# nl1xx/simple-multimodal

Hardware: AMD Instinct MI355X
Metric: fusion fwd+bwd samples/sec at B=16 d=768 (higher is better)
Workload: dtype bf16

## Files before the change

simple-multimodal_amd/csrc/gemm7.hip:

```cpp
#include <algorithm>
#include <vector>
#include "gemm6_parts.h"

namespace {

constexpr int BK = 32, NS = 4;
constexpr int TILE = 256 * BK * 2, PPO = BK / 8;
template <int TN> struct Form {
  static constexpr int BNT = 64 * TN, TILE_B = BNT * BK * 2, STAGE = TILE + TILE_B, PPB = TN, PPW = PPO + PPB;
  static constexpr int LDS = NS * STAGE + 4 * 8192;
};
static_assert(Form<4>::LDS == 160 * 1024 && Form<3>::LDS == 144 * 1024, "LDS of the two forms");

typedef int i32x4_t __attribute__((ext_vector_type(4)));

struct TileSrc {
  const unsigned short* Ab;
  const unsigned short* Bb;
  int recA, recB, stepB, KT;
};
struct TileDst {
  int pi, m0, n0;
};

__device__ __forceinline__ int to_sgpr(int x) {
  int r;
  asm volatile("s_nop 0\n\tv_readfirstlane_b32 %0, %1\n\ts_nop 4" : "=s"(r) : "v"(x));
  return r;
}

template <bool B_KR, int TN>
__device__ __forceinline__ void locate_tile(const GemmArgs& args, const int total_tiles, const int orig, TileSrc& s, TileDst& d, int& lda, int& ldb) {
  const int bid = to_sgpr(mmf_xcd_tile(orig, total_tiles, args.xcd_granule));
  int pi = 0;
  while (pi + 1 < args.nprob && bid >= args.tile_start[pi + 1]) ++pi;
  const mmf_gemm_problem& P = args.p[pi];
  int m0, n0;
  tile_origin<Form<TN>::BNT>(P, bid - args.tile_start[pi], m0, n0);
  m0 = to_sgpr(m0);
  n0 = to_sgpr(n0);
  d.pi = pi; d.m0 = m0; d.n0 = n0;
  lda = P.lda; ldb = P.ldb;
  s.Ab = static_cast<const unsigned short*>(P.A) + (size_t)m0 * P.lda;
  s.Bb = static_cast<const unsigned short*>(P.B) + (B_KR ? (size_t)n0 : (size_t)n0 * P.ldb);
  s.recA = (int)(((long)(P.M - m0 - 1) * P.lda + P.K) * 2);
  s.recB = (int)((B_KR ? ((long)(P.K - 1) * P.ldb + (P.N - n0)) : ((long)(P.N - n0 - 1) * P.ldb + P.K)) * 2);
  s.stepB = (B_KR ? BK * P.ldb : BK) * 2;
  s.KT = P.K / BK;
}

template <int CT, int TN>
__device__ __forceinline__ void drain_tile(const GemmArgs& args, const int pi, const mmf_gemm_problem& P, const int mb, const int nb,
                                           f32x16_t (&acc)[TN][4], char* region, const int lane) {
  constexpr bool AUX = (CT & (MMF_EPI_MASK_AUX | MMF_EPI_ADD_AUX)) != 0;
  constexpr bool DROP = (CT & MMF_EPI_DROPOUT) != 0;
  const unsigned drop_key = DROP ? mmf_rng_key(*args.rng_state, args.site, (unsigned)args.orig[pi]) : 0u;
  const float drop_scale = DROP ? 1.f / (1.f - (float)args.drop_thresh * (1.f / 4294967296.f)) : 1.f;
  const float alpha = (CT & MMF_EPI_MASK_AUX) ? args.alpha : 1.f;
  const int r = lane & 31, h = lane >> 5, q = lane >> 4, cq = lane & 15;
  const unsigned wr_base = (unsigned)(r * 256 + 8 * h + 16 * (r & 15));
  const unsigned rd_base = (unsigned)(q * 256 + ((cq ^ q) << 4));
  auto acc_at = [&](int c) { return region + (wr_base ^ (unsigned)(c << 4)); };
  auto row_at = [&](int it) { return region + it * 1024 + (rd_base ^ (unsigned)((it & 3) << 6)); };
  const bool col_ok = cq < 4 * TN && nb + 8 * cq < P.N;
  const __amdgpu_buffer_rsrc_t crs = __builtin_amdgcn_make_buffer_rsrc(P.C, 0, (int)((((long)P.M - 1) * P.ldc + P.N) * 2), 0x00020000);
  const __amdgpu_buffer_rsrc_t ars = __builtin_amdgcn_make_buffer_rsrc(const_cast<void*>(AUX ? P.aux : P.C), 0,
                                                                       AUX ? (int)((((long)P.M - 1) * P.ldaux + P.N) * 2) : 0, 0x00020000);
  const unsigned c_off0 = col_ok ? (unsigned)(((long)(mb + q) * P.ldc + nb + 8 * cq) * 2) : 0x80000000u;
  const unsigned a_off0 = col_ok ? (unsigned)(((long)(mb + q) * P.ldaux + nb + 8 * cq) * 2) : 0x80000000u;
  const unsigned c_row4 = (unsigned)(4 * P.ldc * 2), a_row4 = (unsigned)(4 * P.ldaux * 2);

  u32x4_t auxr[2][8];
  auto load_aux = [&](int tm, int slot) {
#pragma unroll
    for (int it = 0; it < 8; ++it)
      auxr[slot][it] = __builtin_bit_cast(u32x4_t, __builtin_amdgcn_raw_buffer_load_b128(ars, a_off0 + (unsigned)(8 * tm + it) * a_row4, 0, 0));
  };
  if constexpr (AUX) { load_aux(0, 0); load_aux(1, 1); }
#pragma unroll
  for (int tm = 0; tm < 4; ++tm) {
    u32x2_t axv[TN][4];
    if constexpr (AUX) {
#pragma unroll
      for (int it = 0; it < 8; ++it) *reinterpret_cast<u32x4_t*>(row_at(it)) = auxr[tm & 1][it];
#pragma unroll
      for (int tn = 0; tn < TN; ++tn)
#pragma unroll
        for (int g = 0; g < 4; ++g) axv[tn][g] = *reinterpret_cast<const u32x2_t*>(acc_at(4 * tn + g));
      __builtin_amdgcn_sched_barrier(0);
      if (tm + 2 < 4) load_aux(tm + 2, tm & 1);
      __builtin_amdgcn_sched_barrier(0);
    }
#pragma unroll
    for (int tn = 0; tn < TN; ++tn) {
      asm volatile("" : "+a"(acc[tn][tm]));
#pragma unroll
      for (int g = 0; g < 4; ++g) {
        f32x4_t v = {acc[tn][tm][4 * g], acc[tn][tm][4 * g + 1], acc[tn][tm][4 * g + 2], acc[tn][tm][4 * g + 3]};
        if constexpr (CT & MMF_EPI_RELU) {
#pragma unroll
          for (int e = 0; e < 4; ++e) v[e] = fmaxf(v[e], 0.f);
        }
        if constexpr (DROP) {
          const unsigned idx = (unsigned)(mb + 32 * tm + r) * (unsigned)P.N + (unsigned)(nb + 32 * tn + 8 * g + 4 * h);
#pragma unroll
          for (int e = 0; e < 4; ++e) v[e] = mmf_keep(drop_key, idx + e, args.drop_thresh) ? v[e] * drop_scale : 0.f;
        }
        if constexpr (AUX) {
          const u32x2_t a = axv[tn][g];
          const float a0 = bf16lo(a[0]), a1 = bf16hi(a[0]), a2 = bf16lo(a[1]), a3 = bf16hi(a[1]);
          if constexpr (CT & MMF_EPI_MASK_AUX) {
            v[0] = a0 > 0.f ? v[0] * alpha : 0.f; v[1] = a1 > 0.f ? v[1] * alpha : 0.f;
            v[2] = a2 > 0.f ? v[2] * alpha : 0.f; v[3] = a3 > 0.f ? v[3] * alpha : 0.f;
          } else {
            v[0] += a0; v[1] += a1; v[2] += a2; v[3] += a3;
          }
        }
        *reinterpret_cast<u32x2_t*>(acc_at(4 * tn + g)) = u32x2_t{pack_bf16x2(v[0], v[1]), pack_bf16x2(v[2], v[3])};
      }
      __builtin_amdgcn_sched_barrier(0);
    }
    u32x4_t w[8];
#pragma unroll
    for (int it = 0; it < 8; ++it) w[it] = *reinterpret_cast<const u32x4_t*>(row_at(it));
#pragma unroll
    for (int it = 0; it < 8; ++it) __builtin_amdgcn_raw_buffer_store_b128(w[it], crs, c_off0 + (unsigned)(8 * tm + it) * c_row4, 0, 0);
    __builtin_amdgcn_sched_barrier(0);
  }
}

template <bool B_KR, int CT, int TN>
__device__ __forceinline__ void gemm7_body(const GemmArgs& args, const int total_tiles, char* smem) {
  constexpr bool A_KR = false;
  using F = Form<TN>;
  constexpr int BNT = F::BNT, STAGE = F::STAGE, PPW = F::PPW, NMF = 4 * TN, NRD = 4 + TN;
  constexpr int WA = BK, WB = B_KR ? BNT : BK;

  const int tid = threadIdx.x, lane = tid & 63;
  const int wave = __builtin_amdgcn_readfirstlane(tid >> 6);
  const int wm = wave >> 1, wn = wave & 1;
  const int nwg = gridDim.x;
  const int wid = blockIdx.x;
  auto walk = [&](int round) { return round * nwg + ((round & 1) ? nwg - 1 - wid : wid); };
  int round = 0;
  int orig = walk(0);
  TileSrc ns;
  TileDst cd, nd;
  int KT, lda, ldb;
  locate_tile<B_KR, TN>(args, total_tiles, orig, ns, cd, lda, ldb);
  KT = ns.KT;

  unsigned voff[PPW], voffn[PPW];
  auto set_voff = [&](unsigned (&v)[PPW], int la, int lb) {
#pragma unroll
    for (int i = 0; i < PPO; ++i) v[i] = piece_voff<A_KR, BK>(wave + 4 * i, la, lane);
#pragma unroll
    for (int i = 0; i < TN; ++i) v[PPO + i] = piece_voff<B_KR, BK, BNT>(wave + 4 * i, lb, lane);
  };
  set_voff(voff, lda, ldb);
  char* const my_pieces = smem + wave * 1024;

  struct Desc { int lo, hi, rec; };
  auto mkdesc = [](const unsigned short* p, int rec) {
    const unsigned long long a = (unsigned long long)(uintptr_t)p;
    return Desc{(int)(unsigned)a, (int)((unsigned)(a >> 32) & 0xffffu), rec};
  };
  auto advance = [](Desc& d, int bytes) {
    const unsigned long long a = (((unsigned long long)(unsigned)d.hi << 32) | (unsigned)d.lo) + (unsigned long long)bytes;
    d.lo = (int)(unsigned)a; d.hi = (int)(unsigned)(a >> 32);
    int r;
    asm("s_sub_i32 %0, %1, %2\n\ts_max_i32 %0, %0, 0" : "=s"(r) : "s"(d.rec), "s"(bytes) : "scc");
    d.rec = r;
  };
  Desc dA = mkdesc(ns.Ab, ns.recA);
  Desc dB = mkdesc(ns.Bb, ns.recB);
  constexpr int stepA = BK * 2;
  int stepB = ns.stepB;
  const unsigned lds_pieces = (unsigned)(uintptr_t)(const __attribute__((address_space(3))) char*)my_pieces;
  auto hot_piece = [&](auto ic, const unsigned ring_base) {
    constexpr int I = decltype(ic)::value, OFF = I < PPO ? I * 4096 : TILE + (I - PPO) * 4096;
    const Desc& d = I < PPO ? dA : dB;
    const i32x4_t q = {d.lo, d.hi, d.rec, 0x00020000};
    int m0w;
    asm volatile("s_add_i32 %0, %1, %4\n\ts_nop 0\n\tbuffer_load_dwordx4 %2, %3, 0 offen lds" : "={m0}"(m0w) : "s"(ring_base), "v"(voff[I]), "s"(q), "n"(OFF) : "memory");
    __builtin_amdgcn_sched_barrier(0);
  };

#pragma unroll
  for (int s = 0; s < NS; ++s) {
    const unsigned rb = lds_pieces + (unsigned)(s * STAGE);
    hot_piece(std::integral_constant<int, 0>{}, rb); hot_piece(std::integral_constant<int, 1>{}, rb);
    hot_piece(std::integral_constant<int, 2>{}, rb); hot_piece(std::integral_constant<int, 3>{}, rb);
    if (s + 1 < NS) {
      hot_piece(std::integral_constant<int, 4>{}, rb); hot_piece(std::integral_constant<int, 5>{}, rb);
      hot_piece(std::integral_constant<int, 6>{}, rb);
      if constexpr (TN == 4) hot_piece(std::integral_constant<int, 7>{}, rb);
      advance(dA, stepA); advance(dB, stepB);
    }
  }

  bool has_next = walk(1) < total_tiles;
  nd = cd;
  if (has_next) {
    int la, lb;
    locate_tile<B_KR, TN>(args, total_tiles, walk(1), ns, nd, la, lb);
    set_voff(voffn, la, lb);
  } else {
    ns.recA = 0; ns.recB = 0; ns.stepB = 0;
#pragma unroll
    for (int i = 0; i < PPW; ++i) voffn[i] = voff[i];
  }

  unsigned la0, la1, lb0, lb1;
  Frag4<A_KR>::lane_parts(WA, lane, la0, la1);
  Frag4<B_KR>::lane_parts(WB, lane, lb0, lb1);
  const unsigned smem_base = (unsigned)(uintptr_t)(const __attribute__((address_space(3))) char*)smem;
  const unsigned qa = (unsigned)((WA / 32) * 2048 * 4 * wm);
  const unsigned qb = (unsigned)(B_KR ? 512 * TN * wn : (WB / 32) * 2048 * TN * wn);
  la0 += smem_base + qa; la1 += smem_base + qa;
  lb0 += smem_base + TILE + qb; lb1 += smem_base + TILE + qb;

  f32x16_t acc[TN][4];

  constexpr bool use_bias = (CT & MMF_EPI_BIAS) != 0;
  float bcur[TN] = {};
  auto load_bias = [&](float (&b)[TN], const TileDst& d) {
    const mmf_gemm_problem& P = args.p[d.pi];
    const __amdgpu_buffer_rsrc_t brs = __builtin_amdgcn_make_buffer_rsrc(const_cast<float*>(P.bias), 0, P.N * 4, 0x00020000);
    const unsigned off = (unsigned)((d.n0 + 32 * TN * wn + (lane & 31)) * 4);
#pragma unroll
    for (int tn = 0; tn < TN; ++tn)
      b[tn] = __uint_as_float((unsigned)__builtin_amdgcn_raw_buffer_load_b32(brs, off + (unsigned)(32 * tn * 4), 0, 0));
  };
  auto split3 = [&](float x) {
    const bool lo = lane < 32;
    const unsigned hh = __float_as_uint(x) & 0xffff0000u;
    const float r1 = x - __uint_as_float(hh);
    const unsigned mm = __float_as_uint(r1) & 0xffff0000u;
    const float r2 = r1 - __uint_as_float(mm);
    const unsigned ll = __float_as_uint(r2) & 0xffff0000u;
    const u32x4_t w = {lo ? ((hh >> 16) | mm) : 0u, lo ? (ll >> 16) : 0u, 0u, 0u};
    return __builtin_bit_cast(bf16x8_t, w);
  };
  auto bias_init = [&](const float (&b)[TN]) {
    const f32x16_t zero = {0.f, 0.f, 0.f, 0.f, 0.f, 0.f, 0.f, 0.f, 0.f, 0.f, 0.f, 0.f, 0.f, 0.f, 0.f, 0.f};
    const u32x4_t ow = {lane < 32 ? 0x3f803f80u : 0u, lane < 32 ? 0x00003f80u : 0u, 0u, 0u};
    u32x4_t ones[4] = {ow, ow, ow, ow};
#pragma unroll
    for (int tm = 0; tm < 4; ++tm) asm volatile("" : "+v"(ones[tm]));
#pragma unroll
    for (int tn = 0; tn < TN; ++tn) {
      u32x4_t bw = __builtin_bit_cast(u32x4_t, use_bias ? split3(b[tn]) : __builtin_bit_cast(bf16x8_t, u32x4_t{0u, 0u, 0u, 0u}));
      asm volatile("" : "+v"(bw));
#pragma unroll
      for (int tm = 0; tm < 4; ++tm) {
        acc[tn][tm] = __builtin_amdgcn_mfma_f32_32x32x16_bf16(__builtin_bit_cast(bf16x8_t, bw), __builtin_bit_cast(bf16x8_t, ones[tm]), zero, 0, 0, 0);
        __builtin_amdgcn_sched_barrier(0);
      }
    }
  };
  if constexpr (use_bias) load_bias(bcur, cd);

  vm_wait<PPW * (NS - 2) + PPO>();
  __builtin_amdgcn_s_barrier();
  Frag4<A_KR> fa[2];
  Frag4<B_KR, TN> fb[2];
  fa[0].template issue<WA, 0, 0>(la0, la1);
  fb[0].template issue<WB, 0, 0>(lb0, lb1);
  frag_wait(fa[0], fb[0]);

  auto mf = [&](const Frag4<A_KR>& a, const Frag4<B_KR, TN>& b, int i) {
    const int tm = i / TN, tn = i % TN;
    acc[tn][tm] = __builtin_amdgcn_mfma_f32_32x32x16_bf16(b.get(tn), a.get(tm), acc[tn][tm], 0, 0, 0);
    asm volatile("" ::"a"(acc[tn][tm]));
    __builtin_amdgcn_sched_barrier(0);
  };
#define MMF_G7_READ(dstA, dstB, G, u, so)                                                              \
  do {                                                                                                 \
    if ((u) == 0) dstA.template issue1<WA, G, 0, 0>(la0 + (so), la1 + (so));                            \
    if ((u) == 1) dstA.template issue1<WA, G, 0, 1>(la0 + (so), la1 + (so));                            \
    if ((u) == 2) dstA.template issue1<WA, G, 0, 2>(la0 + (so), la1 + (so));                            \
    if ((u) == 3) dstA.template issue1<WA, G, 0, 3>(la0 + (so), la1 + (so));                            \
    if ((u) == 4) dstB.template issue1<WB, G, 0, 0>(lb0 + (so), lb1 + (so));                            \
    if ((u) == 5) dstB.template issue1<WB, G, 0, 1>(lb0 + (so), lb1 + (so));                            \
    if ((u) == 6) dstB.template issue1<WB, G, 0, 2>(lb0 + (so), lb1 + (so));                            \
    if constexpr (TN == 4) { if ((u) == 7) dstB.template issue1<WB, G, 0, TN - 1>(lb0 + (so), lb1 + (so)); } \
    __builtin_amdgcn_sched_barrier(0);                                                                 \
  } while (0)

  auto stage = [&](const unsigned g, const int kt, const int ksw) {
    unsigned long long swmask;
    const Desc nA = mkdesc(ns.Ab, ns.recA), nB = mkdesc(ns.Bb, ns.recB);
    const unsigned so = (g % NS) * STAGE;
    const unsigned ring_cur = lds_pieces + so, ring_prev = lds_pieces + ((g + NS - 1) % NS) * STAGE;
#pragma unroll
    for (int i = 0; i < NMF; ++i) {
      mf(fa[0], fb[0], i);
      if (i < NRD) MMF_G7_READ(fa[1], fb[1], 1, i, so);
      if (i == NRD)     hot_piece(std::integral_constant<int, 4>{}, ring_prev);
      if (i == NRD + 2) hot_piece(std::integral_constant<int, 5>{}, ring_prev);
      if (i == NRD + 4) hot_piece(std::integral_constant<int, 6>{}, ring_prev);
      if constexpr (TN == 4) { if (i == NRD + 6) hot_piece(std::integral_constant<int, 7>{}, ring_prev); }
    }
    frag_wait(fa[1], fb[1]);
    const unsigned sn = ((g + 1) % NS) * STAGE;
#pragma unroll
    for (int i = 0; i < 4; ++i) mf(fa[1], fb[1], i);
    vm_wait<PPW * (NS - 2)>();
    __builtin_amdgcn_s_barrier();
    __builtin_amdgcn_sched_barrier(0);
#pragma unroll
    for (int i = 4; i < NMF; ++i) {
      mf(fa[1], fb[1], i);
      if (i < 4 + NRD) MMF_G7_READ(fa[0], fb[0], 0, i - 4, sn);
      if (i == 4) {
        advance(dA, stepA);
        advance(dB, stepB);
        asm volatile("" ::"s"(dA.lo), "s"(dA.hi), "s"(dA.rec), "s"(dB.lo), "s"(dB.hi), "s"(dB.rec));
        __builtin_amdgcn_sched_barrier(0);
      }
      if (i == 5) {
        asm volatile("s_cmp_eq_u32 %8, %16\n\t"
                     "s_cselect_b32 %0, %9, %0\n\ts_cselect_b32 %1, %10, %1\n\ts_cselect_b32 %2, %11, %2\n\t"
                     "s_cselect_b32 %3, %12, %3\n\ts_cselect_b32 %4, %13, %4\n\ts_cselect_b32 %5, %14, %5\n\t"
                     "s_cselect_b32 %6, %15, %6\n\ts_cselect_b64 %7, -1, 0"
                     : "+s"(dA.lo), "+s"(dA.hi), "+s"(dA.rec), "+s"(dB.lo), "+s"(dB.hi), "+s"(dB.rec), "+s"(stepB), "=s"(swmask)
                     : "s"(kt), "s"(nA.lo), "s"(nA.hi), "s"(nA.rec), "s"(nB.lo), "s"(nB.hi), "s"(nB.rec), "s"(ns.stepB), "s"(ksw)
                     : "scc");
        __builtin_amdgcn_sched_barrier(0);
      }
      if (i == 6) {
        asm volatile("v_cndmask_b32_e64 %0, %0, %4, %8\n\tv_cndmask_b32_e64 %1, %1, %5, %8\n\t"
                     "v_cndmask_b32_e64 %2, %2, %6, %8\n\tv_cndmask_b32_e64 %3, %3, %7, %8"
                     : "+v"(voff[0]), "+v"(voff[1]), "+v"(voff[2]), "+v"(voff[3])
                     : "v"(voffn[0]), "v"(voffn[1]), "v"(voffn[2]), "v"(voffn[3]), "s"(swmask));
        __builtin_amdgcn_sched_barrier(0);
      }
      if (i == 7) {
        if constexpr (TN == 4)
          asm volatile("v_cndmask_b32_e64 %0, %0, %4, %8\n\tv_cndmask_b32_e64 %1, %1, %5, %8\n\t"
                       "v_cndmask_b32_e64 %2, %2, %6, %8\n\tv_cndmask_b32_e64 %3, %3, %7, %8"
                       : "+v"(voff[4]), "+v"(voff[5]), "+v"(voff[6]), "+v"(voff[7])
                       : "v"(voffn[4]), "v"(voffn[5]), "v"(voffn[6]), "v"(voffn[7]), "s"(swmask));
        else
          asm volatile("v_cndmask_b32_e64 %0, %0, %3, %6\n\tv_cndmask_b32_e64 %1, %1, %4, %6\n\t"
                       "v_cndmask_b32_e64 %2, %2, %5, %6"
                       : "+v"(voff[4]), "+v"(voff[5]), "+v"(voff[6])
                       : "v"(voffn[4]), "v"(voffn[5]), "v"(voffn[6]), "s"(swmask));
        __builtin_amdgcn_sched_barrier(0);
      }
      if (i == NMF - 4) hot_piece(std::integral_constant<int, 0>{}, ring_cur);
      if (i == NMF - 3) hot_piece(std::integral_constant<int, 1>{}, ring_cur);
      if (i == NMF - 2) hot_piece(std::integral_constant<int, 2>{}, ring_cur);
      if (i == NMF - 1) hot_piece(std::integral_constant<int, 3>{}, ring_cur);
    }
    frag_wait(fa[0], fb[0]);
  };

  char* const region = smem + NS * STAGE + wave * 8192;
  unsigned g = 0;
  for (;;) {
    bias_init(bcur);
    const int ksw = KT - NS;
    for (int kt = 0; kt < KT; ++kt, ++g) stage(g, kt, ksw);
    const mmf_gemm_problem& P = args.p[cd.pi];
    const int mb = cd.m0 + 128 * wm, nb = cd.n0 + 32 * TN * wn;
    if constexpr (use_bias) { if (has_next) load_bias(bcur, nd); }
#ifndef MMF_G7_NODRAIN
    drain_tile<CT & ~MMF_EPI_BIAS, TN>(args, cd.pi, P, mb, nb, acc, region, lane);
#else
    if (lane == 0 && mb == -1) static_cast<volatile unsigned short*>(P.C)[0] = (unsigned short)acc[0][0][0];
#endif
    if (!has_next) break;
    ++round;
    orig = walk(round);
    cd = nd;
    KT = ns.KT;
    has_next = walk(round + 1) < total_tiles;
    if (has_next) {
      int la, lb;
      locate_tile<B_KR, TN>(args, total_tiles, walk(round + 1), ns, nd, la, lb);
      set_voff(voffn, la, lb);
    } else {
      ns.recA = 0; ns.recB = 0; ns.stepB = 0;
    }
  }
  vm_wait<0>();
#undef MMF_G7_READ
}

template <bool B_KR, int CT, int TN>
__global__ __launch_bounds__(NTHREADS, 1)
void gemm7_persistent_kernel(const GemmArgs args, const int total_tiles) {
  __shared__ __attribute__((aligned(1024))) char smem[Form<TN>::LDS];
  gemm7_body<B_KR, CT, TN>(args, total_tiles, smem);
}

template <bool B_KR, int CT>
void launch7(const GemmArgs& a, int total, int grid, int tile_n, hipStream_t s) {
  if (tile_n == 192) hipLaunchKernelGGL((gemm7_persistent_kernel<B_KR, CT, 3>), dim3(grid), dim3(NTHREADS), 0, s, a, total);
  else               hipLaunchKernelGGL((gemm7_persistent_kernel<B_KR, CT, 4>), dim3(grid), dim3(NTHREADS), 0, s, a, total);
}
bool launch7_select(int layout, int eflags, const GemmArgs* a, int total, int grid, hipStream_t s, int tile_n = 256) {
  if (layout == MMF_GEMM_NT) {
    if (eflags == 0)                                      { if (a) launch7<false, 0>(*a, total, grid, tile_n, s); return true; }
    if (eflags == MMF_EPI_BIAS)                           { if (a) launch7<false, MMF_EPI_BIAS>(*a, total, grid, tile_n, s); return true; }
    if (eflags == (MMF_EPI_BIAS | MMF_EPI_RELU))          { if (a) launch7<false, MMF_EPI_BIAS | MMF_EPI_RELU>(*a, total, grid, tile_n, s); return true; }
    if (eflags == (MMF_EPI_BIAS | MMF_EPI_ADD_AUX))       { if (a) launch7<false, MMF_EPI_BIAS | MMF_EPI_ADD_AUX>(*a, total, grid, tile_n, s); return true; }
    if (eflags == (MMF_EPI_BIAS | MMF_EPI_RELU | MMF_EPI_DROPOUT)) {
      if (a) launch7<false, MMF_EPI_BIAS | MMF_EPI_RELU | MMF_EPI_DROPOUT>(*a, total, grid, tile_n, s);
      return true;
    }
  } else if (layout == MMF_GEMM_NN) {
    if (eflags == 0)                                      { if (a) launch7<true, 0>(*a, total, grid, tile_n, s); return true; }
    if (eflags == MMF_EPI_MASK_AUX)                       { if (a) launch7<true, MMF_EPI_MASK_AUX>(*a, total, grid, tile_n, s); return true; }
    if (eflags == MMF_EPI_ADD_AUX)                        { if (a) launch7<true, MMF_EPI_ADD_AUX>(*a, total, grid, tile_n, s); return true; }
  }
  return false;
}
}

static int g_persistent_wgs = [] { const char* e = getenv("MMF_GEMM7_WGS"); const int v = e ? atoi(e) : 0; return v > 0 ? v : 0; }();
extern "C" int mmf_gemm_set_persistent_workgroups(int n) {
  if (n < 0 || n > 65536) MMF_FAIL(MMF_E_SHAPE, "mmf_gemm_set_persistent_workgroups: %d not in 0..65536", n);
  g_persistent_wgs = n;
  return MMF_OK;
}
static int g_tile_n = 0;
static thread_local int t_last_tile_n = 0;
extern "C" int mmf_gemm7_set_tile_n(int n) {
  if (n != 0 && n != 256 && n != 192) MMF_FAIL(MMF_E_SHAPE, "mmf_gemm7_set_tile_n: %d is not 0, 256 or 192", n);
  g_tile_n = n;
  return MMF_OK;
}
extern "C" int mmf_gemm7_last_tile_n(void) { return t_last_tile_n; }

namespace {
int persistent_grid_cap() {
  static const int cus = [] { int c = mmf_device_cu_count(); return c > 0 ? c : 256; }();
  return g_persistent_wgs > 0 ? g_persistent_wgs : cus;
}
int tiles_of(const mmf_gemm_problem& p, int bn) { return ((p.M + BM - 1) / BM) * ((p.N + bn - 1) / bn); }
long long walk_makespan(const mmf_gemm_problem* problems, const int* order, int n, int bn, int cap, int granule) {
  int start[MMF_GEMM_MAX_PROBLEMS + 1];
  start[0] = 0;
  for (int i = 0; i < n; ++i) start[i + 1] = start[i] + tiles_of(problems[order[i]], bn);
  const int total = start[n], grid = total < cap ? total : cap;
  if (total == 0) return 0;
  static thread_local std::vector<long long> load;
  load.assign(grid, 0);
  for (int o = 0; o < total; ++o) {
    const int round = o / grid, pos = o % grid, wid = (round & 1) ? grid - 1 - pos : pos;
    const int bid = mmf_xcd_tile(o, total, granule);
    const int pi = (int)(std::upper_bound(start, start + n + 1, bid) - start) - 1;
    load[wid] += (long long)problems[order[pi]].K * bn;
  }
  return *std::max_element(load.begin(), load.end());
}
struct TileNMemo {
  int cap, granule, n, width;
  int mnk[3 * MMF_GEMM_MAX_PROBLEMS];
};
int pick_tile_n(const mmf_gemm_problem* problems, const int* order, int n, int cap) {
  const int granule = mmf_xcd_granule();
  static thread_local TileNMemo memo[16];
  static thread_local int used = 0, next = 0;
  TileNMemo key;
  key.cap = cap; key.granule = granule; key.n = n;
  for (int i = 0; i < n; ++i) {
    const mmf_gemm_problem& p = problems[order[i]];
    key.mnk[3 * i] = p.M; key.mnk[3 * i + 1] = p.N; key.mnk[3 * i + 2] = p.K;
  }
  for (int e = 0; e < used; ++e) {
    const TileNMemo& m = memo[e];
    if (m.cap == cap && m.granule == granule && m.n == n && std::equal(key.mnk, key.mnk + 3 * n, m.mnk)) return m.width;
  }
  key.width = walk_makespan(problems, order, n, 192, cap, granule) < walk_makespan(problems, order, n, 256, cap, granule) ? 192 : 256;
  memo[next] = key;
  next = (next + 1) % 16;
  if (used < 16) ++used;
  return key.width;
}
void sort_by_k(const mmf_gemm_problem* problems, int n, int* order) {
  for (int i = 0; i < n; ++i) order[i] = i;
  std::stable_sort(order, order + n, [&](int x, int y) { return problems[x].K > problems[y].K; });
}
}

extern "C" int mmf_gemm7_tile_n(const mmf_gemm_problem* problems, int num_problems, int workgroups) {
  if (!problems || num_problems < 1 || num_problems > MMF_GEMM_MAX_PROBLEMS || workgroups < 0)
    MMF_FAIL(MMF_E_SHAPE, "mmf_gemm7_tile_n: %d problems, %d workgroups", num_problems, workgroups);
  int order[MMF_GEMM_MAX_PROBLEMS];
  sort_by_k(problems, num_problems, order);
  return pick_tile_n(problems, order, num_problems, workgroups > 0 ? workgroups : persistent_grid_cap());
}

bool mmf_gemm7_supports(const mmf_gemm_problem* problems, int num_problems, int layout, int epilogue, int out_f32, const mmf_gemm_extra* extra) {
  if (out_f32 || !launch7_select(layout, epilogue, nullptr, 0, 0, nullptr)) return false;
  if (extra && extra->alpha != 1.f && !(layout == MMF_GEMM_NN && epilogue == MMF_EPI_MASK_AUX)) return false;
  if ((epilogue & MMF_EPI_DROPOUT) && !(extra && extra->rng_state)) return false;
  for (int i = 0; i < num_problems; ++i) {
    const mmf_gemm_problem& p = problems[i];
    if (p.K % BK || p.K < (NS + 1) * BK || (p.N & 7) || (p.ldc & 7) || (p.aux && ((p.ldaux & 7) || !mmf_aligned16(p.aux)))) return false;
  }
  return true;
}

int mmf_gemm7_launch(const mmf_gemm_problem* problems, int num_problems, int layout, int epilogue,
                     int out_f32, const mmf_gemm_extra* extra, hipStream_t s) {
  if (!mmf_gemm7_supports(problems, num_problems, layout, epilogue, out_f32, extra))
    MMF_FAIL(MMF_E_UNSUPPORTED, "mmf_gemm_grouped: the persistent kernel takes NT / NN launches with bf16 output, K %% 32 == 0, K >= %d, N and the "
             "leading dimensions of C / aux multiples of 8, and the flag sets of the fusion step (alpha only with the NN ReLU mask)", (NS + 1) * BK);
  GemmArgs a;
  a.nprob = num_problems;
  a.epi = epilogue;
  a.xcd_granule = mmf_xcd_granule();
  a.alpha = extra ? extra->alpha : 1.f;
  a.drop_thresh = (extra && (epilogue & MMF_EPI_DROPOUT)) ? mmf_drop_thresh(extra->dropout_p) : 0u;
  a.site = extra ? extra->site : 0u;
  a.rng_state = extra ? reinterpret_cast<const unsigned long long*>(extra->rng_state) : nullptr;
  int total = 0;
  int order[MMF_GEMM_MAX_PROBLEMS];
  sort_by_k(problems, num_problems, order);
  const int cap = persistent_grid_cap();
  const int tile_n = g_tile_n ? g_tile_n : pick_tile_n(problems, order, num_problems, cap);
  for (int i = 0; i < num_problems; ++i) {
    const mmf_gemm_problem& p = problems[order[i]];
    const size_t a_bytes = (size_t)p.M * p.lda * 2;
    const size_t b_bytes = (size_t)(layout == MMF_GEMM_NT ? p.N : p.K) * p.ldb * 2;
    const size_t c_bytes = (size_t)p.M * p.ldc * 2, x_bytes = p.aux ? (size_t)p.M * p.ldaux * 2 : 0;
    if (a_bytes >= 0x7fffffffull || b_bytes >= 0x7fffffffull || c_bytes >= 0x7fffffffull || x_bytes >= 0x7fffffffull)
      MMF_FAIL(MMF_E_UNSUPPORTED, "mmf_gemm_grouped[%d]: operand larger than 2 GiB", i);
    a.tile_start[i] = total;
    total += tiles_of(p, tile_n);
    a.p[i] = p;
    a.orig[i] = (short)order[i];
  }
  a.tile_start[num_problems] = total;
  const int grid = total < cap ? total : cap;
  t_last_tile_n = tile_n;
  launch7_select(layout, epilogue, &a, total, grid, s, tile_n);
  MMF_CHECK_LAUNCH("mmf_gemm_grouped(v7)");
  return MMF_OK;
}
```

Baseline: 7482.

## Overlap next tile's bias-init and first MFMAs with the epilogue drain

Splits the per-tile bias initialization into per-fragment MFMA steps. As each accumulator row block is drained to LDS and global memory, the matching accumulators for the next tile are re-initialized and given their first k-step MFMA. The first stage of each tile is specialized to finish the remaining row block. This hides the drain's store and pack latency under matrix work and removes the serialized bias_init at tile start. In exchange it adds scheduling complexity, register pressure, and a dependence on fragment data for the next tile already being resident during the drain.

```diff
diff --git a/simple-multimodal_amd/csrc/gemm7.hip b/simple-multimodal_amd/csrc/gemm7.hip
--- a/simple-multimodal_amd/csrc/gemm7.hip
+++ b/simple-multimodal_amd/csrc/gemm7.hip
@@ -49,9 +49,9 @@
   s.KT = P.K / BK;
 }
 
-template <int CT, int TN>
+template <int CT, int TN, bool OVERLAP, class Under>
 __device__ __forceinline__ void drain_tile(const GemmArgs& args, const int pi, const mmf_gemm_problem& P, const int mb, const int nb,
-                                           f32x16_t (&acc)[TN][4], char* region, const int lane) {
+                                           f32x16_t (&acc)[TN][4], char* region, const int lane, Under&& under) {
   constexpr bool AUX = (CT & (MMF_EPI_MASK_AUX | MMF_EPI_ADD_AUX)) != 0;
   constexpr bool DROP = (CT & MMF_EPI_DROPOUT) != 0;
   const unsigned drop_key = DROP ? mmf_rng_key(*args.rng_state, args.site, (unsigned)args.orig[pi]) : 0u;
@@ -117,6 +117,12 @@
           }
         }
         *reinterpret_cast<u32x2_t*>(acc_at(4 * tn + g)) = u32x2_t{pack_bf16x2(v[0], v[1]), pack_bf16x2(v[2], v[3])};
+        if constexpr (OVERLAP) {
+          if (tm > 0 && (g & 1)) {
+            __builtin_amdgcn_sched_barrier(0);
+            under(tm - 1, tn, g >> 1);
+          }
+        }
       }
       __builtin_amdgcn_sched_barrier(0);
     }
@@ -126,6 +132,12 @@
 #pragma unroll
     for (int it = 0; it < 8; ++it) __builtin_amdgcn_raw_buffer_store_b128(w[it], crs, c_off0 + (unsigned)(8 * tm + it) * c_row4, 0, 0);
     __builtin_amdgcn_sched_barrier(0);
+  }
+  if constexpr (!OVERLAP) {
+#pragma unroll
+    for (int tm = 0; tm < 3; ++tm)
+#pragma unroll
+      for (int tn = 0; tn < TN; ++tn) { under(tm, tn, 0); under(tm, tn, 1); }
   }
 }
 
@@ -232,32 +244,28 @@
     for (int tn = 0; tn < TN; ++tn)
       b[tn] = __uint_as_float((unsigned)__builtin_amdgcn_raw_buffer_load_b32(brs, off + (unsigned)(32 * tn * 4), 0, 0));
   };
-  auto split3 = [&](float x) {
+  u32x2_t bsplit[TN];
+  auto split3 = [&](const float (&b)[TN]) {
     const bool lo = lane < 32;
-    const unsigned hh = __float_as_uint(x) & 0xffff0000u;
-    const float r1 = x - __uint_as_float(hh);
-    const unsigned mm = __float_as_uint(r1) & 0xffff0000u;
-    const float r2 = r1 - __uint_as_float(mm);
-    const unsigned ll = __float_as_uint(r2) & 0xffff0000u;
-    const u32x4_t w = {lo ? ((hh >> 16) | mm) : 0u, lo ? (ll >> 16) : 0u, 0u, 0u};
-    return __builtin_bit_cast(bf16x8_t, w);
-  };
-  auto bias_init = [&](const float (&b)[TN]) {
+#pragma unroll
+    for (int tn = 0; tn < TN; ++tn) {
+      const float x = b[tn];
+      const unsigned hh = __float_as_uint(x) & 0xffff0000u;
+      const float r1 = x - __uint_as_float(hh);
+      const unsigned mm = __float_as_uint(r1) & 0xffff0000u;
+      const float r2 = r1 - __uint_as_float(mm);
+      const unsigned ll = __float_as_uint(r2) & 0xffff0000u;
+      bsplit[tn] = u32x2_t{lo ? ((hh >> 16) | mm) : 0u, lo ? (ll >> 16) : 0u};
+    }
+  };
+  auto next_start = [&](int tn, int tm) {
     const f32x16_t zero = {0.f, 0.f, 0.f, 0.f, 0.f, 0.f, 0.f, 0.f, 0.f, 0.f, 0.f, 0.f, 0.f, 0.f, 0.f, 0.f};
-    const u32x4_t ow = {lane < 32 ? 0x3f803f80u : 0u, lane < 32 ? 0x00003f80u : 0u, 0u, 0u};
-    u32x4_t ones[4] = {ow, ow, ow, ow};
-#pragma unroll
-    for (int tm = 0; tm < 4; ++tm) asm volatile("" : "+v"(ones[tm]));
-#pragma unroll
-    for (int tn = 0; tn < TN; ++tn) {
-      u32x4_t bw = __builtin_bit_cast(u32x4_t, use_bias ? split3(b[tn]) : __builtin_bit_cast(bf16x8_t, u32x4_t{0u, 0u, 0u, 0u}));
-      asm volatile("" : "+v"(bw));
-#pragma unroll
-      for (int tm = 0; tm < 4; ++tm) {
-        acc[tn][tm] = __builtin_amdgcn_mfma_f32_32x32x16_bf16(__builtin_bit_cast(bf16x8_t, bw), __builtin_bit_cast(bf16x8_t, ones[tm]), zero, 0, 0, 0);
-        __builtin_amdgcn_sched_barrier(0);
-      }
-    }
+    u32x4_t ones = {lane < 32 ? 0x3f803f80u : 0u, lane < 32 ? 0x00003f80u : 0u, 0u, 0u};
+    u32x4_t bw = {use_bias ? bsplit[tn][0] : 0u, use_bias ? bsplit[tn][1] : 0u, 0u, 0u};
+    asm volatile("" : "+v"(bw), "+v"(ones));
+    acc[tn][tm] = __builtin_amdgcn_mfma_f32_32x32x16_bf16(__builtin_bit_cast(bf16x8_t, bw), __builtin_bit_cast(bf16x8_t, ones), zero, 0, 0, 0);
+    asm volatile("" ::"a"(acc[tn][tm]));
+    __builtin_amdgcn_sched_barrier(0);
   };
   if constexpr (use_bias) load_bias(bcur, cd);
 
@@ -274,6 +282,15 @@
     acc[tn][tm] = __builtin_amdgcn_mfma_f32_32x32x16_bf16(b.get(tn), a.get(tm), acc[tn][tm], 0, 0, 0);
     asm volatile("" ::"a"(acc[tn][tm]));
     __builtin_amdgcn_sched_barrier(0);
+  };
+  auto next_first = [&](int tn, int tm) {
+    asm volatile("" : "+v"(fa[0].v[tm]));
+    acc[tn][tm] = __builtin_amdgcn_mfma_f32_32x32x16_bf16(fb[0].get(tn), fa[0].get(tm), acc[tn][tm], 0, 0, 0);
+    asm volatile("" ::"a"(acc[tn][tm]));
+    __builtin_amdgcn_sched_barrier(0);
+  };
+  auto under = [&](int tm, int tn, int half) {
+    if (half == 0) next_start(tn, tm); else next_first(tn, tm);
   };
 #define MMF_G7_READ(dstA, dstB, G, u, so)                                                              \
   do {                                                                                                 \
@@ -288,14 +305,17 @@
     __builtin_amdgcn_sched_barrier(0);                                                                 \
   } while (0)
 
-  auto stage = [&](const unsigned g, const int kt, const int ksw) {
+  auto stage = [&](auto first, const unsigned g, const int kt, const int ksw) {
+    constexpr bool FIRST = decltype(first)::value;
     unsigned long long swmask;
     const Desc nA = mkdesc(ns.Ab, ns.recA), nB = mkdesc(ns.Bb, ns.recB);
     const unsigned so = (g % NS) * STAGE;
     const unsigned ring_cur = lds_pieces + so, ring_prev = lds_pieces + ((g + NS - 1) % NS) * STAGE;
 #pragma unroll
     for (int i = 0; i < NMF; ++i) {
-      mf(fa[0], fb[0], i);
+      if constexpr (!FIRST) mf(fa[0], fb[0], i);
+      else if (i < TN) next_start(i, 3);
+      else if (i < 2 * TN) next_first(i - TN, 3);
       if (i < NRD) MMF_G7_READ(fa[1], fb[1], 1, i, so);
       if (i == NRD)     hot_piece(std::integral_constant<int, 4>{}, ring_prev);
       if (i == NRD + 2) hot_piece(std::integral_constant<int, 5>{}, ring_prev);
@@ -359,17 +379,40 @@
 
   char* const region = smem + NS * STAGE + wave * 8192;
   unsigned g = 0;
+  if constexpr (use_bias) split3(bcur);
+#pragma unroll
+  for (int tm = 0; tm < 3; ++tm)
+#pragma unroll
+    for (int tn = 0; tn < TN; ++tn) next_start(tn, tm);
+#pragma unroll
+  for (int tm = 0; tm < 3; ++tm)
+#pragma unroll
+    for (int tn = 0; tn < TN; ++tn) next_first(tn, tm);
+#ifdef MMF_G7_SERIAL_DRAIN
+  constexpr bool OVERLAP = false;
+#else
+  constexpr bool OVERLAP = true;
+#endif
   for (;;) {
-    bias_init(bcur);
     const int ksw = KT - NS;
-    for (int kt = 0; kt < KT; ++kt, ++g) stage(g, kt, ksw);
+    stage(std::true_type{}, g, 0, ksw);
+    ++g;
+    for (int kt = 1; kt < KT; ++kt, ++g) stage(std::false_type{}, g, kt, ksw);
     const mmf_gemm_problem& P = args.p[cd.pi];
     const int mb = cd.m0 + 128 * wm, nb = cd.n0 + 32 * TN * wn;
     if constexpr (use_bias) { if (has_next) load_bias(bcur, nd); }
+    auto under_drain = [&](int tm, int tn, int half) {
+      if constexpr (use_bias) { if (tm == 0 && tn == 0 && half == 0) split3(bcur); }
+      under(tm, tn, half);
+    };
 #ifndef MMF_G7_NODRAIN
-    drain_tile<CT & ~MMF_EPI_BIAS, TN>(args, cd.pi, P, mb, nb, acc, region, lane);
+    drain_tile<CT & ~MMF_EPI_BIAS, TN, OVERLAP>(args, cd.pi, P, mb, nb, acc, region, lane, under_drain);
 #else
     if (lane == 0 && mb == -1) static_cast<volatile unsigned short*>(P.C)[0] = (unsigned short)acc[0][0][0];
+#pragma unroll
+    for (int tm = 0; tm < 3; ++tm)
+#pragma unroll
+      for (int tn = 0; tn < TN; ++tn) { under_drain(tm, tn, 0); under_drain(tm, tn, 1); }
 #endif
     if (!has_next) break;
     ++round;
```

New measurement: 7474. No clear change (-0.1%).
